# MicrobialDarkMatter/nanomotif

Hardware: AMD Instinct MI355X
Metric: motif-sites scored/sec (1 Gbp synthetic metagenome) (higher is better)
Workload: dtype u32 bit-planes / int64 counts

## Files before the change

### nanomotif_amd/csrc/nmscan.hip

```cpp
#define NM_SCORE_KERNEL_SOURCE
#include "nmscan_device.h"

using namespace nmdetail;

namespace {

thread_local std::string g_err;

__global__ __launch_bounds__(256) void pack_kernel(const uint8_t *__restrict__ ascii,
                                                   const uint64_t *__restrict__ contig_src,
                                                   const uint64_t *__restrict__ contig_len,
                                                   const uint32_t *__restrict__ chunk_contig,
                                                   const uint32_t *__restrict__ chunk_first,
                                                   uint32_t *__restrict__ H, uint32_t *__restrict__ L,
                                                   uint32_t *__restrict__ V, unsigned long long *__restrict__ other) {
    const uint32_t chunk = blockIdx.x;
    const uint32_t contig = chunk_contig[chunk];
    if (contig == 0xFFFFFFFFu) return;
    const uint64_t beg = contig_src[contig], len = contig_len[contig];
    const uint64_t local0 = (uint64_t)(chunk - chunk_first[contig]) * CHUNK_BP;
    const int lane = threadIdx.x & 63, wave = threadIdx.x >> 6;
    for (int it = wave; it < CHUNK_BP / 64; it += 4) {
        const uint64_t p = local0 + (uint64_t)it * 64 + lane;
        uint8_t c = 0;
// ... 514 lines not shown
    if (rc) return rc;
    c->cur_stage->last_out = r.rq.d_out;
    c->cur_stage->last_stream = r.sst;
    c->last_score_stream = r.sst;
    c->timed = !c->ev_collect && r.timed_launch;
    c->launches += 1;
    c->last_wgs = p.last_wgs;
    c->last_compact = p.all_compact ? p.n_prog : 0;
    c->last_general = p.all_compact ? 0 : p.n_prog;
    if (r.rq.defer) {
        nmdetail::wait_set(c, wait_slot, nm_ctx::Waiting{r.hs + p.off_counts, p.out_bytes, c->cur_stage, true});
    } else if (p.via_stage) {
        HIP_TRY(hipEventSynchronize(c->cur_stage->busy));
        memcpy(r.rq.h_out, r.hs + p.off_counts, p.out_bytes);
    } else if (r.rq.h_out) {
        HIP_TRY(hipMemcpyAsync(r.rq.h_out, r.out, p.out_bytes, hipMemcpyDeviceToHost, c->stream));
        HIP_TRY(hipStreamSynchronize(c->stream));
    }
    return NM_OK;
}

PlanFacts plan_facts(const nm_ctx *c) {
    PlanFacts f;
    f.n_bins = c->n_bins;
    f.bin_nchunks = c->bin_nchunks.data();
    f.bin_chunk0 = c->bin_chunk0.data();
    f.bin_ncontigs = c->bin_ncontigs.data();
    static_assert(NM_MAX_MOD_SLOTS <= 32, "one bit per mod slot");
    for (int sl = 0; sl < NM_MAX_MOD_SLOTS; ++sl) {
        f.slot_present |= (c->slots[sl].present ? 1u : 0u) << sl;
        f.slot_is_c |= (c->slots[sl].canonical == 'C' ? 1u : 0u) << sl;
    }
    f.n_segments = c->n_segments;
    f.seg_chunks = c->seg_chunks;
    f.n_cus = c->n_cus;
    f.opt_no_lit = c->opt_no_lit;
    f.opt_no_cf = c->opt_no_cf;
    f.opt_no_inline = c->opt_no_inline;
    f.opt_fine = c->opt_fine;
    f.opt_split = c->opt_split;
    return f;
}

int score_impl(nm_ctx *c, const ScoreRequest &rq) {
    if (!c) return fail(NM_EINVAL, "ctx is NULL");
    if (!c->dH) return fail(NM_ESTATE, "nm_upload_contigs has not been called");
    nm_ctx::Waiting &wait_slot = rq.spec ? c->spec_wait[rq.flight] : c->score_wait[rq.flight];
    if (rq.defer) {
        if (wait_slot.open) return fail(NM_ESTATE, "nm_score_batch_begin: the previous batch has not been collected (nm_score_batch_end)");
        nmdetail::wait_set(c, wait_slot, nm_ctx::Waiting{nullptr, 0, nullptr, true});
    }
    if (rq.n_cand == 0) return NM_OK;
    HIP_TRY(hipSetDevice(c->device));
    const PlanFacts f = plan_facts(c);
    c->bucket.assign((size_t)NM_MAX_MOD_SLOTS * f.n_bins + 1, 0);
    c->bin_active.assign(f.n_bins, 0);
    ScorePlan p;
    if (plan_classify(p, rq, f, c->bucket.data(), c->bin_active.data())) return fail(p.status, "%s", p.err);
    plan_shape(p, rq, f);
    plan_layout(p, rq);
    int rc = ensure_stage(c, p.via_stage ? p.stage_end : p.total, 1);
    if (rc) return rc;
    ScoreRun r{rq, p};
    r.sst = rq.spec ? static_cast<hipStream_t>(rq.stream) : c->stream;
    r.laned = c->score_lanes == 2 && rq.d_out && !rq.h_out && !rq.defer;
    if (!r.laned && !rq.spec) {
// ... 18 lines not shown
        HIP_TRY(hipStreamSynchronize(c->stream));
        HIP_TRY(hipStreamSynchronize(c->copy_stream));
        HIP_TRY(nmdetail::sync_flight_streams(c));
        rc = join_lanes(c);
        if (rc) return rc;
        if (c->d_programs) (void)nmdetail::dev_free(c->d_programs);
        c->d_programs = nullptr;
        c->prog_cap_dw = 0;
        HIP_TRY(nmdetail::dev_malloc(&c->d_programs, p.prog_dw * 2 * 4 * NM_STAGE_RING));
        c->prog_cap_dw = p.prog_dw * 2;
    }
    r.d_prog = c->d_programs + (size_t)(c->cur_stage - c->stage) * c->prog_cap_dw;
    r.out = rq.spec ? reinterpret_cast<unsigned long long *>(r.ds + p.off_counts) : rq.d_out;
    if (!r.out) {
        if (c->counts_cap < p.out_rows) {
            if (c->d_counts) (void)nmdetail::dev_free(c->d_counts);
            c->d_counts = nullptr;
            c->counts_cap = 0;
            HIP_TRY(nmdetail::dev_malloc(&c->d_counts, (size_t)p.out_rows * 2 * sizeof(unsigned long long) * 2));
            c->counts_cap = (size_t)p.out_rows * 2;
        }
        r.out = c->d_counts;
    }
    rc = score_prepare(c, r, f.slot_is_c);
    if (rc) return rc;
    plan_geometry(p, f);
    ScoreArgs a{};
    a.seq = Planes{c->dH, c->dL, c->dV, c->d_needs_v};
    for (int s = 0; s < NM_MAX_MOD_SLOTS; ++s) {
        const ModSlot &ms = c->slots[s];
        a.st[s] = StatePlanes{ms.planes[0], ms.planes[1], ms.planes[2], ms.planes[3], ms.planes[4], ms.planes[5]};
        a.slot_is_c[s] = ms.canonical == 'C';
    }
    a.segments = p.own_segments ? reinterpret_cast<const uint4 *>(r.ds + p.off_segs) : c->d_segments;
    a.n_segments = p.n_segments;
    a.n_bins = c->n_bins;
    a.programs = r.d_prog;
    a.orig_index = reinterpret_cast<uint32_t *>(r.ds + p.off_orig);
    a.cand_range = reinterpret_cast<uint4 *>(r.ds + p.off_range);
    a.out = r.out;
    a.chunk_rank = c->d_chunk_rank;
    a.row_base = reinterpret_cast<const uint64_t *>(r.ds + p.off_rows);
    for (uint32_t i = 0; i < p.n_active; ++i) a.active_slot[i] = p.active[i];
    a.split_log2 = p.split_log2;
    a.pieces_per_run = p.pieces_per_run;
    a.fine_log2 = p.fine_log2;
    a.j_big = p.j_big;
    const LaunchShape shape{p.any_wide, p.all_compact, p.lit, p.cf, p.fuse, p.per_contig, p.classes};
    if (r.timed_launch && p.compile != PLAN_COMPILE_SPEC) HIP_TRY(hipEventRecord(r.e0, r.sst));
    if (p.n_prog) launch_score(a, p.gx, p.gy, shape, r.sst);
    HIP_TRY(hipGetLastError());
    if (r.timed_launch) HIP_TRY(hipEventRecord(r.e1, r.sst));
    return score_collect(c, r, wait_slot);
}

}

int nm_set_error(int code, const char *fmt, ...) {
    char buf[512];
    va_list ap;
    va_start(ap, fmt);
    vsnprintf(buf, sizeof buf, fmt, ap);
    va_end(ap);
    g_err = buf;
    return code;
}

// ... 33 lines not shown
    HIP_TRY(hipEventCreate(&c->ev0));
    HIP_TRY(hipEventCreate(&c->ev1));
    HIP_TRY(nmdetail::dev_malloc(&c->d_err, sizeof(unsigned int)));
    HIP_TRY(nmdetail::dev_malloc(&c->d_other, sizeof(unsigned long long)));
    return NM_OK;
}

int nm_ctx_create(int device, nm_ctx **out) {
    if (!out) return fail(NM_EINVAL, "out is NULL");
    *out = nullptr;
    int n = 0;
    HIP_TRY(hipGetDeviceCount(&n));
    if (device < 0 || device >= n) return fail(NM_EINVAL, "device %d not in 0..%d", device, n - 1);
    HIP_TRY(hipSetDevice(device));
    nm_ctx *c = new (std::nothrow) nm_ctx();
    if (!c) return fail(NM_ENOMEM, "out of host memory");
    c->device = device;
    c->stream = nullptr;
    nmdetail::g_live_ctx += 1;
    const int rc = ctx_init(c);
    if (rc != NM_OK) {
        const std::string keep = g_err;
        (void)nm_ctx_destroy(c);
        g_err = keep;
        return rc;
    }
    *out = c;
    return NM_OK;
}

static void free_assembly(nm_ctx *c) {
    drop_ingest_rows(c);
    nmdetail::free_readstats(c);
    void *ptrs[] = {c->dH , c->d_needs_v, c->d_contig_chunk, c->d_contig_len, c->d_segments, c->d_chunk_rank};
    c->d_chunk_rank = nullptr;
    for (void *p : ptrs)
        if (p) (void)nmdetail::dev_free(p);
    c->dH = c->dL = c->dV = nullptr;
    c->d_needs_v = nullptr;
    c->d_contig_chunk = nullptr;
    c->d_contig_len = nullptr;
    c->d_segments = nullptr;
    for (int b = 0; b < 4; ++b) {
        if (c->d_rank[b]) (void)nmdetail::dev_free(c->d_rank[b]);
        if (c->d_base_total[b]) (void)nmdetail::dev_free(c->d_base_total[b]);
        c->d_rank[b] = nullptr;
        c->d_base_total[b] = nullptr;
    }
    for (auto &s : c->slots) {
        free_slot_planes(s);
        s.present = false;
        s.n_rows = 0;
        drop_slot_ranks(s);
    }
}

int nm_ctx_destroy(nm_ctx *c) {
    if (!c) return NM_OK;
    (void)hipSetDevice(c->device);
    if (c->stream) (void)hipStreamSynchronize(c->stream);
    if (c->own_stream) (void)hipStreamSynchronize(c->own_stream);
    if (c->copy_stream) (void)hipStreamSynchronize(c->copy_stream);
    if (c->lane_stream) (void)hipStreamSynchronize(c->lane_stream);
    c->lane_pending = false;
    (void)nm_comm_destroy(c);
    free_assembly(c);
    for (auto &st : c->stage) {
        if (st.d) (void)nmdetail::dev_free(st.d);
// ... 138 lines not shown
        guard.tmp[0] = d_ascii;
    }
    HIP_TRY(nmdetail::dev_malloc(&d_off, (size_t)(n_contigs + 1) * 8));
    guard.tmp[1] = d_off;
    HIP_TRY(nmdetail::dev_malloc(&d_chunk_contig, (size_t)c->n_chunks * 4));
    guard.tmp[2] = d_chunk_contig;
    if (!on_device && c->total_bp) HIP_TRY(hipMemcpyAsync(d_ascii, seq_ascii, c->total_bp, hipMemcpyHostToDevice, c->stream));
    HIP_TRY(hipMemcpyAsync(d_off, src_off ? src_off : offsets, (size_t)(n_contigs + (src_off ? 0 : 1)) * 8, hipMemcpyHostToDevice, c->stream));
    HIP_TRY(hipMemcpyAsync(d_chunk_contig, chunk_contig.data(), (size_t)c->n_chunks * 4, hipMemcpyHostToDevice, c->stream));
    {
        std::vector<uint32_t> chunk_rank(c->n_chunks, 0);
        for (uint32_t ch = 0; ch < c->n_chunks; ++ch)
            if (chunk_contig[ch] != 0xFFFFFFFFu) chunk_rank[ch] = c->contig_rank[chunk_contig[ch]];
        HIP_TRY(nmdetail::dev_malloc(&c->d_chunk_rank, (size_t)c->n_chunks * 4));
        HIP_TRY(hipMemcpy(c->d_chunk_rank, chunk_rank.data(), (size_t)c->n_chunks * 4, hipMemcpyHostToDevice));
    }
    HIP_TRY(hipMemsetAsync(c->d_other, 0, sizeof(unsigned long long), c->stream));
    hipLaunchKernelGGL(pack_kernel, dim3(c->n_chunks), dim3(256), 0, c->stream, d_ascii, d_off, c->d_contig_len, d_chunk_contig,
                       c->d_contig_chunk, c->dH, c->dL, c->dV, c->d_other);
    HIP_TRY(hipGetLastError());
    hipLaunchKernelGGL(needs_v_kernel, dim3(c->n_chunks), dim3(CHUNK_WORDS), 0, c->stream, c->dV, c->d_needs_v, c->n_chunks);
    HIP_TRY(hipGetLastError());
    std::vector<uint4> segs;
    for (uint32_t b = 0; b < n_bins; ++b)
        for (uint32_t k = 0; k < c->bin_nchunks[b]; k += c->seg_chunks)
            segs.push_back(make_uint4(c->bin_chunk0[b] + k, std::min<uint32_t>(c->seg_chunks, c->bin_nchunks[b] - k), b, 0));
    c->n_segments = (uint32_t)segs.size();
    HIP_TRY(nmdetail::dev_malloc(&c->d_segments, std::max<size_t>(segs.size(), 1) * sizeof(uint4)));
    if (!segs.empty()) HIP_TRY(hipMemcpyAsync(c->d_segments, segs.data(), segs.size() * sizeof(uint4), hipMemcpyHostToDevice, c->stream));
    unsigned long long other = 0;
    HIP_TRY(hipMemcpyAsync(&other, c->d_other, sizeof other, hipMemcpyDeviceToHost, c->stream));
    HIP_TRY(hipStreamSynchronize(c->stream));
    c->other_letters = other;
    guard.keep = true;
    return NM_OK;
}

static int upload_pileup_impl(nm_ctx *c, uint32_t mod_slot, uint8_t canonical_base, double low, double high,
                              uint64_t n_rows, const uint32_t *contig_id, const uint32_t *position,
                              const uint8_t *strand, const double *fraction_mod, int append, bool on_device) {
    if (!c) return fail(NM_EINVAL, "ctx is NULL");
    if (!c->dH) return fail(NM_ESTATE, "nm_upload_contigs must come first");
    if (mod_slot >= NM_MAX_MOD_SLOTS) return fail(NM_EINVAL, "mod_slot %u >= %d", mod_slot, NM_MAX_MOD_SLOTS);
    if (canonical_base != 'A' && canonical_base != 'C') return fail(NM_EINVAL, "canonical base must be 'A' or 'C'");
    if (!(high > low)) return fail(NM_EINVAL, "high threshold must exceed low (find_motifs_bin.py:117-118)");
    if (n_rows && (!contig_id || !position || !strand || !fraction_mod)) return fail(NM_EINVAL, "NULL column");
    HIP_TRY(hipSetDevice(c->device));
    HIP_TRY(hipStreamSynchronize(c->stream));
    {
        const int rcj = join_lanes(c);
        if (rcj) return rcj;
    }
    ModSlot &ms = c->slots[mod_slot];
    drop_slot_ranks(ms);
    const size_t words = plane_words(c);
    if (!ms.present || !append) {
        HIP_TRY(alloc_slot_planes(ms, words));
        HIP_TRY(hipMemsetAsync(ms.planes[0], 0, words * 4 * 6, c->stream));
        ms.n_rows = 0;
    } else if (ms.canonical != canonical_base || ms.low != low || ms.high != high) {
        return fail(NM_EINVAL, "append with different canonical base / thresholds than the slot holds");
    }
    ms.present = true;
    ms.canonical = canonical_base;
    ms.low = low;
    ms.high = high;
// ... 447 lines not shown
```

### nanomotif_amd/csrc/nmscan_device.h

```cpp
#pragma once
#include "nmscan_internal.h"

namespace nmdetail {

__device__ __forceinline__ uint32_t alignbit(uint32_t hi, uint32_t lo, uint32_t sh) {
    return __builtin_amdgcn_alignbit(hi, lo, sh);
}

typedef const uint32_t __attribute__((address_space(4))) *cu32p;
typedef const uint8_t __attribute__((address_space(4))) *cu8p;

#ifndef NM_LIT_WAVES
#define NM_LIT_WAVES 4
#endif

template <int GN_, int GP_, bool COMPACT_, int NS_, bool LIT_, bool CF_, bool PC_ = false, bool CLS_ = false>
struct Variant {
    static constexpr int GN = GN_, GP = GP_, NS = NS_;
    static constexpr bool COMPACT = COMPACT_, LIT = LIT_, CF = CF_, PC = PC_;
    static constexpr bool CLS = CLS_;
    static_assert(!CLS || (GN == 1 && GP == 1 && COMPACT && NS == 1 && !LIT && !CF), "class planes: narrow compact heavy variants only");
    static constexpr int NW = T_WORDS + GN + GP;
    static constexpr int NP = LIT ? 4 : 8;
    static constexpr int NST = COMPACT ? 2 : 4;
    static constexpr int PDW = (GN + GP) * NP;
};

template <class K>
struct RawChunk {
    uint32_t h[K::NW], l[K::NW], v[K::NW];
    uint32_t s[K::NS][K::NST][T_WORDS];
    bool need_v;

    __device__ __forceinline__ void load(const Planes &seq, const StatePlanes (&stp)[K::NS], uint32_t chunk, int lane) {
        constexpr int GN = K::GN, GP = K::GP;
        need_v = ((cu8p)seq.needs_v)[chunk] != 0;
        const size_t base = (size_t)chunk * CHUNK_WORDS + (size_t)lane * T_WORDS;
#pragma unroll
        for (int j = 0; j < K::NS; ++j) {
            const uint32_t *src[4] = {K::COMPACT ? stp[j].M : stp[j].MP, K::COMPACT ? stp[j].U : stp[j].UP, stp[j].MM, stp[j].UM};
#pragma unroll
            for (int i = 0; i < K::NST; ++i) {
                const uint4 q = *reinterpret_cast<const uint4 *>(src[i] + base);
                s[j][i][0] = q.x; s[j][i][1] = q.y; s[j][i][2] = q.z; s[j][i][3] = q.w;
            }
        }
        const uint4 h4 = *reinterpret_cast<const uint4 *>(seq.H + base);
        const uint4 l4 = *reinterpret_cast<const uint4 *>(seq.L + base);
        h[GN + 0] = h4.x; h[GN + 1] = h4.y; h[GN + 2] = h4.z; h[GN + 3] = h4.w;
        l[GN + 0] = l4.x; l[GN + 1] = l4.y; l[GN + 2] = l4.z; l[GN + 3] = l4.w;
#pragma unroll
        for (int j = 0; j < GN; ++j) { h[j] = seq.H[base - GN + j]; l[j] = seq.L[base - GN + j]; }
#pragma unroll
        for (int j = 0; j < GP; ++j) { h[GN + T_WORDS + j] = seq.H[base + T_WORDS + j]; l[GN + T_WORDS + j] = seq.L[base + T_WORDS + j]; }
        if (need_v) {
            const uint4 v4 = *reinterpret_cast<const uint4 *>(seq.V + base);
            v[GN + 0] = v4.x; v[GN + 1] = v4.y; v[GN + 2] = v4.z; v[GN + 3] = v4.w;
#pragma unroll
            for (int j = 0; j < GN; ++j) v[j] = seq.V[base - GN + j];
#pragma unroll
            for (int j = 0; j < GP; ++j) v[GN + T_WORDS + j] = seq.V[base + T_WORDS + j];
        } else if constexpr (!K::CLS) {
#pragma unroll
            for (int j = 0; j < K::NW; ++j) v[j] = 0xFFFFFFFFu;
        }
    }
};

template <class K>
struct Tile {
// ... 405 lines not shown
                    prog[1] = desc[1];
                }
                r.w = 1;
            }
            r.z = n_prog + g;
        }
    }
    range[g] = r;
}


}

#ifdef NM_SCORE_KERNEL_SOURCE

namespace nmdetail {

struct ScoreArgs {
    Planes seq;
    StatePlanes st[NM_MAX_MOD_SLOTS];
    const uint4 *segments;
    uint32_t n_segments;
    uint32_t split_log2;
    uint32_t pieces_per_run, j_big, fine_log2;
    uint32_t n_bins;
    const uint4 *cand_range;
    const uint32_t *programs;
    const uint32_t *orig_index;
    unsigned long long *out;
    const uint32_t *chunk_rank;
    const uint64_t *row_base;
    uint32_t active_slot[NM_MAX_MOD_SLOTS];
    uint32_t slot_is_c[NM_MAX_MOD_SLOTS];
};

void launch_score_classes(const ScoreArgs &a, uint32_t gx, uint32_t gy, bool per_contig, hipStream_t s);

}

namespace {

using namespace nmdetail;

template <class K, int I = 0>
__device__ __forceinline__ void apply_single(uint32_t idx, uint32_t r, const Tile<K> &tile, const uint32_t (&base)[T_WORDS],
                                             uint32_t (&acc)[T_WORDS]) {
    if constexpr (I < K::PDW) {
        if (idx == I) {
            constexpr int g = I / K::NP, p = I % K::NP;
#pragma unroll
            for (int t = 0; t < T_WORDS; ++t) acc[t] = base[t] & alignbit(tile.w[p][t + g + 1], tile.w[p][t + g], r);
        } else {
            apply_single<K, I + 1>(idx, r, tile, base, acc);
        }
    } else {
#pragma unroll
        for (int t = 0; t < T_WORDS; ++t) acc[t] = base[t];
    }
}

template <class K>
__device__ __forceinline__ void emit_counts(const ScoreArgs &a, uint32_t n_mod, uint32_t n_non, uint32_t k0, uint32_t k,
                                            uint32_t *lds_acc, uint32_t lds_row0, int lane, uint32_t contig_rank) {
    if (K::PC) {
        if constexpr (K::CLS) {
#define NM_SWZ_ADD(o)                                                                         \
// ... 197 lines not shown
            const uint32_t i = idx >> 2, q = idx & 3;
            const uint32_t j = (i >> 1) % NS, k = (i >> 1) / NS;
            uint32_t s = 0;
#pragma unroll 4
            for (int jj = 0; jj < 16; ++jj) s += lds_acc[i * 64 + q * 16 + jj];
            s += __shfl_xor(s, 1);
            s += __shfl_xor(s, 2);
            if (q == 0 && s) {
                uint4 rj = range[0];
#pragma unroll
                for (int t = 1; t < NS; ++t)
                    if (j == (uint32_t)t) rj = range[t];
                if (pass0 + k < rj.y) {
                    const uint32_t orig = a.orig_index[rj.x + pass0 + k];
                    atomicAdd(a.out + (size_t)orig * 2 + (i & 1), (unsigned long long)s);
                }
            }
        }
        __syncthreads();
    };
    uint32_t pass0 = 0;
    if (EARLY) {
        const uint32_t rows_hi = NS * min(H, most);
        clear_rows(rows_hi);
        if (wave < sg.y) score_chunk(first, 0, sg.x + wave);
        for (uint32_t ck = wave + 4; ck < sg.y; ck += 4) {
            RawChunk<K> cur;
            cur.load(a.seq, stp, sg.x + ck, lane);
            score_chunk(cur, 0, sg.x + ck);
        }
        flush_rows(rows_hi, 0);
        pass0 = H;
    }
    for (; pass0 < most; pass0 += H) {
        const uint32_t rows_hi = NS * min(H, most - pass0);
        clear_rows(rows_hi);
        for (uint32_t ck = wave; ck < sg.y; ck += 4) {
            RawChunk<K> cur;
            cur.load(a.seq, stp, sg.x + ck, lane);
            score_chunk(cur, pass0, sg.x + ck);
        }
        flush_rows(rows_hi, pass0);
    }
}

#define NM_SCORE_BOUNDS __launch_bounds__(256, (K::GN + K::GP > 2 ? 2 : (K::LIT ? NM_LIT_WAVES : (K::CLS ? 6 : 4))))

#define NM_SLOT_SETUP                                                                                               \
    const int lane = threadIdx.x & 63;                                                                              \
    const uint32_t wave = __builtin_amdgcn_readfirstlane(threadIdx.x >> 6);  \
    StatePlanes stp[K::NS];                                                                                         \
    bool is_c[K::NS];                                                                                               \
    _Pragma("unroll") for (int j = 0; j < K::NS; ++j) {                                                             \
        const uint32_t slot = a.active_slot[K::NS == 1 ? blockIdx.y : (uint32_t)j];                                 \
        stp[j] = a.st[slot];                                                                                        \
        is_c[j] = a.slot_is_c[slot] != 0;                                                                           \
    }

template <class K>
__global__ NM_SCORE_BOUNDS void score_kernel(ScoreArgs a) {
    __shared__ uint32_t lds_acc[BMAX * 2 * 64];
    const uint32_t lanes_x = K::CF ? 1u : 8u;
    const uint32_t x = K::CF ? 0u : blockIdx.x % 8, j = K::CF ? blockIdx.x : blockIdx.x / 8;
    uint32_t piece, sub = 0, n_sub = 1;
    if (j < a.j_big) piece = x * a.pieces_per_run + j;
    else {
        const uint32_t k = j - a.j_big;
        piece = x * a.pieces_per_run + a.j_big + (k >> a.fine_log2);
        sub = k & ((1u << a.fine_log2) - 1);
        n_sub = 1u << a.fine_log2;
        if (a.j_big + (k >> a.fine_log2) >= a.pieces_per_run) return;
    }
    (void)lanes_x;
    const uint32_t seg = piece >> a.split_log2;
    if (seg >= a.n_segments) return;
    uint4 sg = a.segments[seg];
    sg.x = __builtin_amdgcn_readfirstlane(sg.x);
    sg.y = __builtin_amdgcn_readfirstlane(sg.y);
    sg.z = __builtin_amdgcn_readfirstlane(sg.z);
    if (a.split_log2) {
        const uint32_t len = (sg.y + (1u << a.split_log2) - 1) >> a.split_log2;
        const uint32_t at = (piece & ((1u << a.split_log2) - 1)) * len;
        if (at >= sg.y) return;
        sg.x += at;
        sg.y = min(len, sg.y - at);
    }
    if (n_sub > 1) {
        const uint32_t len = (sg.y + n_sub - 1) / n_sub;
        const uint32_t at = sub * len;
        if (at >= sg.y) return;
        sg.x += at;
        sg.y = min(len, sg.y - at);
    }
    NM_SLOT_SETUP
    score_piece<K>(a, sg, stp, is_c, lds_acc, lane, wave);
}

}

#ifdef NM_SCORE_CLASSES_UNIT
namespace nmdetail {

void launch_score_classes(const ScoreArgs &a, uint32_t gx, uint32_t gy, bool per_contig, hipStream_t s) {
    if (per_contig) hipLaunchKernelGGL((score_kernel<Variant<1, 1, true, 1, false, false, true, true>>), dim3(gx, gy), dim3(256), 0, s, a);
    else hipLaunchKernelGGL((score_kernel<Variant<1, 1, true, 1, false, false, false, true>>), dim3(gx, gy), dim3(256), 0, s, a);
}

}
#endif

#endif
```

### nanomotif_amd/csrc/nmscan_internal.h

```cpp
#pragma once
#include <hip/hip_runtime.h>

#include <algorithm>
#include <cstdarg>
#include <cstdint>
#include <cstdio>
#include <cstring>
#include <functional>
#include <mutex>
#include <numeric>
#include <string>
#include <vector>

#include "../../include/nmscan.h"
#include "nmscore_plan.h"
#include "nmspec.h"

int nm_set_error(int code, const char *fmt, ...);
#define fail nm_set_error

#define HIP_TRY(expr)                                                                                   \
    do {                                                                                                \
        hipError_t e_ = (expr);                                                                         \
        if (e_ != hipSuccess) return fail(NM_EHIP, "%s failed: %s", #expr, hipGetErrorString(e_));      \
    } while (0)

namespace nmdetail {

hipError_t device_alloc(void **p, size_t bytes);
hipError_t device_free(void *p);
template <class T>
inline hipError_t dev_malloc(T **p, size_t bytes) { return device_alloc(reinterpret_cast<void **>(p), bytes); }
inline hipError_t dev_free(void *p) { return device_free(p); }

constexpr int T_WORDS = 4;
constexpr int CHUNK_WORDS = 64 * T_WORDS;
constexpr int CHUNK_BP = CHUNK_WORDS * 32;
constexpr int GAP_BP = 96;
constexpr int SEG_CHUNKS = 16;
constexpr int BMAX = 32;
constexpr int NM_MAX_MOD_CODES = 8;
constexpr int NM_CODE_STRIDE = 128;
constexpr int WIN_MAX_W = NM_WIN_MAX_WIDTH;
constexpr int RANK_BLOCK_WORDS = 16;
constexpr int RANK_PER_CHUNK = CHUNK_WORDS / RANK_BLOCK_WORDS;

struct Planes {
    const uint32_t *H, *L, *V;
// ... 48 lines not shown
    hipStream_t last_score_stream = nullptr;
    std::vector<uint32_t> bucket;
    std::vector<uint8_t> bin_active;
    std::vector<nmdetail::WinTask> win_tasks;
    uint32_t *d_win_planes = nullptr, *d_win_alive = nullptr;
    uint64_t win_planes_cap = 0, win_alive_cap = 0, win_planes_used = 0, win_alive_used = 0;
    nmdetail::WinTask *d_win_tasks = nullptr;
    size_t d_win_tasks_cap = 0;
    bool win_tasks_dirty = false;
    std::vector<uint32_t> ing_kept;
    int ing_slot_of_mod[8] = {-1, -1, -1, -1, -1, -1, -1, -1};
    uint64_t ing_nconf = 0, ing_total_kept = 0, ing_classified = 0;
    uint32_t *d_programs = nullptr;
    size_t prog_cap_dw = 0;
    hipEvent_t ev0 = nullptr, ev1 = nullptr;
    bool timed = false;
    std::vector<std::pair<hipEvent_t, hipEvent_t>> ev_pool;
    size_t ev_used = 0;
    bool ev_collect = false;
    bool busy_open = false;
    bool ev_collect_all = false;
    uint32_t n_contigs = 0, n_bins = 0, n_chunks = 0;
    uint64_t total_bp = 0;
    std::vector<uint64_t> contig_len;
    std::vector<uint32_t> contig_chunk, contig_bin, contig_nchunks;
    std::vector<uint32_t> bin_chunk0, bin_nchunks, bin_ncontigs, contig_rank;
    uint32_t *d_chunk_rank = nullptr;
    uint32_t *dH = nullptr, *dL = nullptr, *dV = nullptr;
    uint8_t *d_needs_v = nullptr;
    uint32_t *d_contig_chunk = nullptr;
    uint64_t *d_contig_len = nullptr;
    uint4 *d_segments = nullptr;
    uint32_t n_segments = 0;
    nmdetail::ModSlot slots[NM_MAX_MOD_SLOTS];
    nmdetail::ReadStats readstats[NM_MAX_MOD_SLOTS];
    uint32_t *d_chunk_contig = nullptr;
    struct Stage {
        void *d = nullptr, *h = nullptr;
        size_t bytes = 0;
        hipEvent_t busy = nullptr;
        bool pending = false;
        const void *last_out = nullptr;
        hipStream_t last_stream = nullptr;
    } stage[NM_STAGE_SLOTS];
    int stage_next = 0;
    int stage_next_deep = 0;
    void *d_stage = nullptr, *h_stage = nullptr;
    Stage *cur_stage = nullptr;
    struct Waiting {
        const void *h = nullptr;
        size_t bytes = 0;
        Stage *stage = nullptr;
        bool open = false;
    } score_wait[NM_FLIGHTS], win_wait[NM_FLIGHTS], spec_wait[NM_FLIGHTS];
    std::mutex wait_mu;
    hipStream_t flight_stream[NM_FLIGHTS - 1] = {};
    double *d_spec_bg = nullptr;
    uint32_t spec_tasks = 0, spec_width = 0;
    unsigned long long *d_spec_counts[NM_FLIGHTS] = {}, *d_flight_counts[NM_FLIGHTS] = {};
    size_t spec_counts_cap[NM_FLIGHTS] = {}, flight_counts_cap[NM_FLIGHTS] = {};
    unsigned long long *d_counts = nullptr;
    size_t counts_cap = 0;
    unsigned int *d_err = nullptr;
    uint32_t *d_rank[4] = {nullptr, nullptr, nullptr, nullptr};
    uint64_t *d_base_total[4] = {nullptr, nullptr, nullptr, nullptr};
    unsigned long long *d_other = nullptr;
// ... 121 lines not shown
```

### nanomotif_amd/csrc/nmscore_plan.h

```cpp
#pragma once
#include <algorithm>
#include <cstdarg>
#include <cstddef>
#include <cstdint>
#include <cstdio>
#include <cstdlib>
#include <cstring>

#include "../../include/nmscan.h"

namespace nmdetail {

struct SpecSource;

struct CandRec {
    uint32_t mask_off;
    uint32_t orig;
    uint8_t len, modpos, slot, pad;
};

struct PlanU4 { uint32_t x, y, z, w; };

constexpr size_t PLAN_STAGE_DIRECT_MAX = (size_t)4 << 20;

struct ScoreRequest {
    uint32_t n_cand = 0;
    const uint32_t *bin = nullptr;
    const uint8_t *slot = nullptr, *len = nullptr, *modpos = nullptr;
    const uint32_t *mask_off = nullptr;
    const uint8_t *masks = nullptr;
    unsigned long long *d_out = nullptr;
    int64_t *h_out = nullptr;
    const uint64_t *row_offset = nullptr;
    bool defer = false;
    const SpecSource *spec = nullptr;
    uint32_t spec_mask_stride = 0;
    size_t spec_extra_in = 0, spec_extra_out = 0;
    void *stream = nullptr;
    int flight = 0;
};

struct PlanFacts {
    uint32_t n_bins = 0;
    const uint32_t *bin_nchunks = nullptr, *bin_chunk0 = nullptr, *bin_ncontigs = nullptr;
    uint32_t slot_present = 0, slot_is_c = 0;
    uint32_t n_segments = 0, seg_chunks = 16, n_cus = 256;
    bool opt_no_lit = false, opt_no_cf = false, opt_no_inline = false;
    int opt_fine = -1, opt_split = -1;
};

enum PlanCompile { PLAN_COMPILE_NONE, PLAN_COMPILE_FUSED, PLAN_COMPILE_ONLY, PLAN_COMPILE_THEN_COMMON, PLAN_COMPILE_SPEC };

struct ScorePlan {
    int status = NM_OK;
    char err[192] = {0};
    int any_wide = 0;
    bool all_compact = true, all_literal = true, per_contig = false;
    uint32_t n_prog = 0;
    uint64_t mask_lo = 0, mask_hi = 0;
    uint32_t n_active = 0, active[NM_MAX_MOD_SLOTS] = {};
    int slot_to_active[NM_MAX_MOD_SLOTS] = {};
    uint32_t n_active_bins = 0, n_groups = 0;
    size_t n_active_segs = 0;
    uint64_t out_rows = 0;
    bool lit = false, light = false, cf = false, classes = false, cls_head = true, fuse = false;
    bool own_segments = false, via_stage = false, inline_prep = false, by_kernels = false;
    PlanCompile compile = PLAN_COMPILE_NONE;
    uint32_t np = 8, pdw = 0, n_entries = 0;
    size_t prog_dw = 0;
    size_t off_orig = 0, off_masks = 0, off_range = 0, off_rows = 0, off_segs = 0, off_posof = 0, off_xin = 0, total = 0;
    size_t off_counts = 0, off_xout = 0, stage_end = 0;
    size_t range_bytes = 0, out_bytes = 0, clear_bytes = 0;
    uint32_t n_segments = 0;
    uint32_t split_log2 = 0, pieces_per_run = 0, fine_log2 = 0, j_big = 0, gx = 0, gy = 1;
    uint64_t last_wgs = 0;
};

inline size_t plan_align16(size_t x) { return (x + 15) & ~(size_t)15; }

inline int plan_fail(ScorePlan &p, int code, const char *fmt, ...) __attribute__((format(printf, 3, 4)));
inline int plan_fail(ScorePlan &p, int code, const char *fmt, ...) {
    va_list ap;
    va_start(ap, fmt);
    vsnprintf(p.err, sizeof p.err, fmt, ap);
    va_end(ap);
    return p.status = code;
}

inline int check_motif(ScorePlan &p, uint32_t k, uint32_t len, uint32_t mp, const uint8_t *m, uint32_t max_len, bool *literal) {
    if (len == 0 || len > max_len) return plan_fail(p, NM_ERANGE, "candidate %u: motif length %u outside 1..%d", k, len, (int)max_len);
    if (mp >= len) return plan_fail(p, NM_EINVAL, "candidate %u: mod_position %u outside motif of length %u", k, mp, len);
    uint32_t all_and = 15u, any_zero = 0, any_set = 0;
    for (uint32_t j = 0; j < len; ++j) {
        const uint32_t v = m[j] & 15u;
        all_and &= v;
        any_zero |= (v == 0);
        any_set |= (v != 15u) & ((v & (v - 1)) != 0);
    }
    if (any_zero) return plan_fail(p, NM_EINVAL, "candidate %u: empty base set in the motif", k);
    if (all_and == 15u) return plan_fail(p, NM_EINVAL, "candidate %u: motif has no specified position", k);
    *literal = !any_set;
    return NM_OK;
}

inline uint32_t number_active_slots(const bool used[NM_MAX_MOD_SLOTS], int slot_to_active[NM_MAX_MOD_SLOTS], uint32_t *active = nullptr) {
    uint32_t n = 0;
    for (int s = 0; s < NM_MAX_MOD_SLOTS; ++s) {
        slot_to_active[s] = -1;
        if (!used[s]) continue;
        if (active) active[n] = (uint32_t)s;
        slot_to_active[s] = (int)n++;
    }
    return n;
}

inline int plan_classify(ScorePlan &p, const ScoreRequest &rq, const PlanFacts &f, uint32_t *bucket, uint8_t *bin_active) {
    const uint32_t n_bins = f.n_bins;
    uint64_t mask_bytes = 0, mask_lo = ~0ull;
    bool slot_used[NM_MAX_MOD_SLOTS] = {};
    for (uint32_t k = 0; k < rq.n_cand; ++k) {
        const uint32_t slot = rq.slot[k], bin = rq.bin[k];
        if (slot >= NM_MAX_MOD_SLOTS || !(f.slot_present >> slot & 1u))
            return plan_fail(p, NM_ESTATE, "candidate %u uses mod slot %u with no pileup uploaded", k, slot);
        if (bin >= n_bins) return plan_fail(p, NM_EINVAL, "candidate %u: bin %u >= n_bins %u", k, bin, n_bins);
        if (f.bin_nchunks[bin] == 0) continue;
        if (rq.spec) {
            mask_lo = 0;
            mask_bytes = std::max<uint64_t>(mask_bytes, (uint64_t)(k + 1) * rq.spec_mask_stride);
        } else {
            const uint32_t len = rq.len[k], mp = rq.modpos[k];
            const uint8_t *m = rq.masks + rq.mask_off[k];
            bool literal = true;
            if (check_motif(p, k, len, mp, m, NM_MAX_MOTIF_LEN, &literal)) return p.status;
            if (!literal) p.all_literal = false;
            mask_lo = std::min<uint64_t>(mask_lo, rq.mask_off[k]);
            mask_bytes = std::max<uint64_t>(mask_bytes, (uint64_t)rq.mask_off[k] + len);
            const uint32_t reach = std::max(mp, len - 1 - mp);
            if (reach > 95) return plan_fail(p, NM_ERANGE, "candidate %u: a position %u away from the modified base (the engine reaches 95)", k, reach);
            p.any_wide = std::max(p.any_wide, reach > 63 ? 2 : reach > 31 ? 1 : 0);
            if ((m[mp] & 15u) != ((f.slot_is_c >> slot & 1u) ? NM_BASE_C : NM_BASE_A)) p.all_compact = false;
        }
        bucket[(size_t)slot * n_bins + bin + 1] += 1;
        slot_used[slot] = true;
        p.n_prog += 1;
    }
    if (p.n_prog == 0) { mask_lo = 0; mask_bytes = 0; }
    p.mask_lo = mask_lo;
    p.mask_hi = mask_bytes;
    p.n_active = number_active_slots(slot_used, p.slot_to_active, p.active);
    p.per_contig = rq.row_offset != nullptr;
    p.out_rows = p.per_contig ? rq.row_offset[rq.n_cand] : rq.n_cand;
    if (p.per_contig)
        for (uint32_t k = 0; k < rq.n_cand; ++k)
            if (rq.row_offset[k + 1] - rq.row_offset[k] != f.bin_ncontigs[rq.bin[k]])
                return plan_fail(p, NM_EINVAL, "candidate %u: %llu output rows for a bin of %u resident contigs", k,
                                 (unsigned long long)(rq.row_offset[k + 1] - rq.row_offset[k]), f.bin_ncontigs[rq.bin[k]]);
    for (uint32_t b = 0; b < n_bins; ++b) {
        uint32_t groups = 0;
        for (uint32_t i = 0; i < p.n_active; ++i) groups += bucket[(size_t)p.active[i] * n_bins + b + 1] > 0;
        if (!groups) continue;
        p.n_groups += groups;
        bin_active[b] = 1;
        p.n_active_bins += 1;
        p.n_active_segs += (f.bin_nchunks[b] + f.seg_chunks - 1) / f.seg_chunks;
    }
    return NM_OK;
}

inline void plan_shape(ScorePlan &p, const ScoreRequest &rq, const PlanFacts &f) {
    p.lit = p.all_literal && p.all_compact && !p.any_wide && !f.opt_no_lit && !p.per_contig;
    p.np = p.lit ? 4u : 8u;
    p.pdw = 2u * (2u + 2u * (uint32_t)p.any_wide) * p.np;
    p.light = (uint64_t)p.n_prog <= 6ull * p.n_groups && !p.per_contig;
    p.cf = p.light && !f.opt_no_cf;
    p.fuse = p.n_active == 2 && p.cf && p.lit;
    const char *cls_env = getenv("NM_SCORE_CLASSES"), *head_env = getenv("NM_SCORE_HEAD");
    p.cls_head = !(head_env && atoi(head_env) == 0);
    p.classes = !rq.spec && !p.lit && !p.any_wide && p.all_compact && !p.cf && !(cls_env && atoi(cls_env) == 0);
    p.own_segments = p.n_prog && p.n_active_segs * 4 <= (size_t)f.n_segments * 3 && getenv("NM_ALL_SEGMENTS") == nullptr;
    p.n_segments = p.own_segments ? (uint32_t)p.n_active_segs : f.n_segments;
    p.n_entries = std::max(p.n_active, 1u) * f.n_bins;
    p.prog_dw = ((size_t)std::max(p.n_prog, 1u) + (p.cf ? p.n_entries : 0)) * p.pdw;
    p.out_bytes = (size_t)p.out_rows * 2 * sizeof(int64_t);
    p.via_stage = rq.defer || (rq.h_out && p.out_bytes <= PLAN_STAGE_DIRECT_MAX);
    p.inline_prep = (rq.h_out || rq.defer) && !f.opt_no_inline;
    if (rq.spec) p.compile = PLAN_COMPILE_SPEC;
    else if (!p.n_prog) p.compile = PLAN_COMPILE_NONE;
    else if (p.cf && p.n_prog <= 2048 && p.n_entries <= 8192 && !f.opt_no_inline) p.compile = PLAN_COMPILE_FUSED;
    else p.compile = p.cf ? PLAN_COMPILE_THEN_COMMON : PLAN_COMPILE_ONLY;
}

inline void plan_layout(ScorePlan &p, const ScoreRequest &rq) {
    const size_t rec_bytes = (size_t)p.n_prog * sizeof(CandRec);
    p.off_orig = plan_align16(rec_bytes);
    p.off_masks = plan_align16(p.off_orig + (size_t)p.n_prog * 4);
    p.off_range = plan_align16(p.off_masks + (p.mask_hi - p.mask_lo));
    p.range_bytes = (size_t)p.n_entries * sizeof(PlanU4);
    p.off_rows = plan_align16(p.off_range + p.range_bytes);
    const size_t rows_end = p.off_rows + (p.per_contig ? (size_t)p.n_prog * 8 : 0);
    p.off_segs = plan_align16(rows_end);
    const size_t segs_end = p.own_segments ? p.off_segs + p.n_active_segs * sizeof(PlanU4) : p.off_segs;
    p.off_posof = plan_align16(segs_end);
    p.off_xin = plan_align16(p.off_posof + (size_t)rq.n_cand * 4);
    p.total = rq.spec ? p.off_xin + rq.spec_extra_in : p.own_segments ? segs_end : rows_end;
    p.off_counts = plan_align16(p.total);
    p.off_xout = plan_align16(p.off_counts + p.out_bytes);
    p.stage_end = rq.spec ? p.off_xout + rq.spec_extra_out : p.off_counts + p.out_bytes;
    p.clear_bytes = rq.spec ? p.stage_end - p.off_counts : (size_t)p.out_rows * 2 * sizeof(unsigned long long);
    p.by_kernels = p.inline_prep && p.total <= PLAN_STAGE_DIRECT_MAX && (p.via_stage || !rq.h_out) && getenv("NM_STAGE_COPIES") == nullptr;
}

inline void plan_fill(const ScorePlan &p, const ScoreRequest &rq, const PlanFacts &f, uint32_t *bucket, const uint8_t *bin_active, uint8_t *hs) {
    const uint32_t n_bins = f.n_bins;
    CandRec *h_rec = reinterpret_cast<CandRec *>(hs);
    uint32_t *h_orig = reinterpret_cast<uint32_t *>(hs + p.off_orig);
    PlanU4 *h_range = reinterpret_cast<PlanU4 *>(hs + p.off_range);
    if (!rq.spec && p.mask_hi > p.mask_lo) memcpy(hs + p.off_masks, rq.masks + p.mask_lo, p.mask_hi - p.mask_lo);
    memset(h_range, 0, p.range_bytes);
    if (p.own_segments) {
        PlanU4 *h_segs = reinterpret_cast<PlanU4 *>(hs + p.off_segs);
        size_t at = 0;
        for (uint32_t b = 0; b < n_bins; ++b)
            if (bin_active[b])
                for (uint32_t k = 0; k < f.bin_nchunks[b]; k += f.seg_chunks)
                    h_segs[at++] = PlanU4{f.bin_chunk0[b] + k, std::min<uint32_t>(f.seg_chunks, f.bin_nchunks[b] - k), b, 0};
    }
    const size_t n_bucket = (size_t)NM_MAX_MOD_SLOTS * n_bins + 1;
    for (size_t i = 1; i < n_bucket; ++i) bucket[i] += bucket[i - 1];
    for (uint32_t i = 0; i < p.n_active; ++i)
        for (uint32_t b = 0; b < n_bins; ++b) {
            const uint32_t lo = bucket[(size_t)p.active[i] * n_bins + b], hi = bucket[(size_t)p.active[i] * n_bins + b + 1];
            if (hi > lo) h_range[(size_t)i * n_bins + b] = PlanU4{lo, hi - lo, 0xFFFFFFFFu, 0};
        }
    for (uint32_t k = 0; k < rq.n_cand; ++k) {
        const uint32_t slot = rq.slot[k], bin = rq.bin[k];
        if (f.bin_nchunks[bin] == 0) continue;
        const uint32_t at = bucket[(size_t)slot * n_bins + bin]++;
        h_orig[at] = k;
        if (rq.spec) {
            h_rec[at] = CandRec{k * rq.spec_mask_stride, k, 0, 0, (uint8_t)slot, 0};
            reinterpret_cast<uint32_t *>(hs + p.off_posof)[k] = at;
            continue;
        }
        h_rec[at] = CandRec{(uint32_t)(rq.mask_off[k] - p.mask_lo), k, rq.len[k], rq.modpos[k], (uint8_t)slot, 0};
        if (p.per_contig) reinterpret_cast<uint64_t *>(hs + p.off_rows)[at] = rq.row_offset[k];
    }
}

inline void plan_geometry(ScorePlan &p, const PlanFacts &f) {
    uint64_t est_wgs = (uint64_t)p.n_segments * p.n_groups / std::max<uint32_t>(p.own_segments ? p.n_active_bins : f.n_bins, 1);
    if (p.light && p.n_active == 2 && p.lit) est_wgs = (est_wgs + 1) / 2;
    const uint64_t resident = (uint64_t)f.n_cus * 6;
    uint32_t split_log2 = 0;
    while (split_log2 < 2 && (est_wgs << split_log2) < 2 * resident) ++split_log2;
    if (f.opt_split >= 0) split_log2 = (uint32_t)f.opt_split;
    p.split_log2 = split_log2;
    const uint32_t runs = p.cf ? 1u : 8u;
    const uint32_t n_pieces = p.n_segments << split_log2;
// ... 12 lines not shown
```

Before: 102900 billion.

## Score chunks through a prebuilt work list that packs partial contig tails

At upload time a work list is built for each bin. It drops chunks lying wholly in contig padding and, by default, packs the partially filled tail chunks of short contigs into dense 64-strip rows, with one strip per lane. The non-CF, non-per-contig scoring path reads each chunk through this list, indirecting per lane for packed rows, so waves stop scanning empty bit-plane padding. The cost is an extra host-side build and a device allocation at upload, plus one more indirection in the kernel. Packed rows force need_v on, and segment geometry now depends on the list.

```diff
diff --git a/nanomotif_amd/csrc/nmscan.hip b/nanomotif_amd/csrc/nmscan.hip
--- a/nanomotif_amd/csrc/nmscan.hip
+++ b/nanomotif_amd/csrc/nmscan.hip
@@ -570,6 +570,11 @@
         f.slot_is_c |= (c->slots[sl].canonical == 'C' ? 1u : 0u) << sl;
     }
     f.n_segments = c->n_segments;
+    for (int w = 0; w < 2; ++w) {
+        f.list_start[w] = c->list_start[w].data();
+        f.list_len[w] = c->list_len[w].data();
+        f.list_segments[w] = c->n_list_segments[w];
+    }
     f.seg_chunks = c->seg_chunks;
     f.n_cus = c->n_cus;
     f.opt_no_lit = c->opt_no_lit;
@@ -654,7 +659,9 @@
         a.st[s] = StatePlanes{ms.planes[0], ms.planes[1], ms.planes[2], ms.planes[3], ms.planes[4], ms.planes[5]};
         a.slot_is_c[s] = ms.canonical == 'C';
     }
-    a.segments = p.own_segments ? reinterpret_cast<const uint4 *>(r.ds + p.off_segs) : c->d_segments;
+    a.segments = p.own_segments ? reinterpret_cast<const uint4 *>(r.ds + p.off_segs) : p.use_list ? c->d_list_segments[p.pack] : c->d_segments;
+    a.work_list = c->d_work_list[p.pack];
+    a.strip_rows = c->d_strip_rows;
     a.n_segments = p.n_segments;
     a.n_bins = c->n_bins;
     a.programs = r.d_prog;
@@ -754,8 +761,17 @@
 static void free_assembly(nm_ctx *c) {
     drop_ingest_rows(c);
     nmdetail::free_readstats(c);
-    void *ptrs[] = {c->dH , c->d_needs_v, c->d_contig_chunk, c->d_contig_len, c->d_segments, c->d_chunk_rank};
+    void *ptrs[] = {c->dH , c->d_needs_v, c->d_contig_chunk, c->d_contig_len, c->d_segments, c->d_chunk_rank,
+                    c->d_work_list[0] };
     c->d_chunk_rank = nullptr;
+    for (int w = 0; w < 2; ++w) {
+        c->d_work_list[w] = nullptr;
+        c->d_list_segments[w] = nullptr;
+        c->n_list_segments[w] = 0;
+        c->list_start[w].clear();
+        c->list_len[w].clear();
+    }
+    c->d_strip_rows = nullptr;
     for (void *p : ptrs)
         if (p) (void)nmdetail::dev_free(p);
     c->dH = c->dL = c->dV = nullptr;
@@ -960,6 +976,33 @@
     HIP_TRY(hipMemcpyAsync(&other, c->d_other, sizeof other, hipMemcpyDeviceToHost, c->stream));
     HIP_TRY(hipStreamSynchronize(c->stream));
     c->other_letters = other;
+    {
+        std::vector<uint8_t> needs_v(c->n_chunks);
+        HIP_TRY(hipMemcpy(needs_v.data(), c->d_needs_v, c->n_chunks, hipMemcpyDeviceToHost));
+        WorkList wl[2];
+        for (int w = 0; w < 2; ++w)
+            build_work_list(wl[w], w == 1, n_bins, n_contigs, order.data(), c->contig_bin.data(), c->contig_len.data(), c->contig_chunk.data(), needs_v.data(),
+                            c->n_chunks, c->seg_chunks);
+        const size_t o_list[2] = {0, wl[0].entries.size()}, o_strips = o_list[1] + wl[1].entries.size();
+        const size_t o_segs0 = (o_strips + wl[1].strip_rows.size() + 3) & ~(size_t)3, o_segs1 = o_segs0 + wl[0].segs.size() * 4;
+        const size_t o_segs[2] = {o_segs0, o_segs1}, total = o_segs1 + wl[1].segs.size() * 4;
+        std::vector<uint32_t> blob(std::max<size_t>(total, 4), 0);
+        for (int w = 0; w < 2; ++w) {
+            std::copy(wl[w].entries.begin(), wl[w].entries.end(), blob.begin() + o_list[w]);
+            if (!wl[w].segs.empty()) memcpy(blob.data() + o_segs[w], wl[w].segs.data(), wl[w].segs.size() * sizeof(PlanU4));
+        }
+        std::copy(wl[1].strip_rows.begin(), wl[1].strip_rows.end(), blob.begin() + o_strips);
+        HIP_TRY(nmdetail::dev_malloc(&c->d_work_list[0], blob.size() * 4));
+        HIP_TRY(hipMemcpy(c->d_work_list[0], blob.data(), blob.size() * 4, hipMemcpyHostToDevice));
+        c->d_work_list[1] = c->d_work_list[0] + o_list[1];
+        c->d_strip_rows = c->d_work_list[0] + o_strips;
+        for (int w = 0; w < 2; ++w) {
+            c->d_list_segments[w] = reinterpret_cast<uint4 *>(c->d_work_list[0] + o_segs[w]);
+            c->n_list_segments[w] = (uint32_t)wl[w].segs.size();
+            c->list_start[w] = std::move(wl[w].bin_start);
+            c->list_len[w] = std::move(wl[w].bin_len);
+        }
+    }
     guard.keep = true;
     return NM_OK;
 }
diff --git a/nanomotif_amd/csrc/nmscan_device.h b/nanomotif_amd/csrc/nmscan_device.h
--- a/nanomotif_amd/csrc/nmscan_device.h
+++ b/nanomotif_amd/csrc/nmscan_device.h
@@ -33,9 +33,21 @@
     bool need_v;
 
     __device__ __forceinline__ void load(const Planes &seq, const StatePlanes (&stp)[K::NS], uint32_t chunk, int lane) {
+        need_v = ((cu8p)seq.needs_v)[chunk] != 0;
+        load_at(seq, stp, (size_t)chunk * CHUNK_WORDS + (size_t)lane * T_WORDS);
+    }
+    __device__ __forceinline__ void load_entry(const Planes &seq, const StatePlanes (&stp)[K::NS], uint32_t entry, const uint32_t *strip_rows, int lane) {
+        if (entry & WORK_PACKED) {
+            const uint32_t w = strip_rows[(size_t)(entry & ~WORK_PACKED) * WORK_STRIPS + lane];
+            need_v = true;
+            load_at(seq, stp, (size_t)(w == WORK_NO_STRIP ? (uint32_t)T_WORDS : w));
+        } else {
+            need_v = (entry & WORK_NEED_V) != 0;
+            load_at(seq, stp, (size_t)(entry & (WORK_NEED_V - 1)) * CHUNK_WORDS + (size_t)lane * T_WORDS);
+        }
+    }
+    __device__ __forceinline__ void load_at(const Planes &seq, const StatePlanes (&stp)[K::NS], const size_t base) {
         constexpr int GN = K::GN, GP = K::GP;
-        need_v = ((cu8p)seq.needs_v)[chunk] != 0;
-        const size_t base = (size_t)chunk * CHUNK_WORDS + (size_t)lane * T_WORDS;
 #pragma unroll
         for (int j = 0; j < K::NS; ++j) {
             const uint32_t *src[4] = {K::COMPACT ? stp[j].M : stp[j].MP, K::COMPACT ? stp[j].U : stp[j].UP, stp[j].MM, stp[j].UM};
@@ -507,6 +519,8 @@
     const uint64_t *row_base;
     uint32_t active_slot[NM_MAX_MOD_SLOTS];
     uint32_t slot_is_c[NM_MAX_MOD_SLOTS];
+    const uint32_t *work_list;
+    const uint32_t *strip_rows;
 };
 
 void launch_score_classes(const ScoreArgs &a, uint32_t gx, uint32_t gy, bool per_contig, hipStream_t s);
@@ -770,13 +784,15 @@
         flush_rows(rows_hi, 0);
         pass0 = H;
     }
+    constexpr bool LIST = !K::CF && !K::PC;
     for (; pass0 < most; pass0 += H) {
         const uint32_t rows_hi = NS * min(H, most - pass0);
         clear_rows(rows_hi);
         for (uint32_t ck = wave; ck < sg.y; ck += 4) {
             RawChunk<K> cur;
-            cur.load(a.seq, stp, sg.x + ck, lane);
-            score_chunk(cur, pass0, sg.x + ck);
+            if constexpr (LIST) cur.load_entry(a.seq, stp, ((cu32p)a.work_list)[sg.x + ck], a.strip_rows, lane);
+            else cur.load(a.seq, stp, sg.x + ck, lane);
+            score_chunk(cur, pass0, LIST ? 0u : sg.x + ck);
         }
         flush_rows(rows_hi, pass0);
     }
@@ -798,38 +814,20 @@
 template <class K>
 __global__ NM_SCORE_BOUNDS void score_kernel(ScoreArgs a) {
     __shared__ uint32_t lds_acc[BMAX * 2 * 64];
-    const uint32_t lanes_x = K::CF ? 1u : 8u;
-    const uint32_t x = K::CF ? 0u : blockIdx.x % 8, j = K::CF ? blockIdx.x : blockIdx.x / 8;
-    uint32_t piece, sub = 0, n_sub = 1;
-    if (j < a.j_big) piece = x * a.pieces_per_run + j;
+    const PlanGrid grid{a.n_segments, a.split_log2, a.pieces_per_run, a.j_big, a.fine_log2};
+    uint32_t piece, sub, n_sub;
+    if (!plan_block_piece(grid, K::CF, blockIdx.x, &piece, &sub, &n_sub)) return;
+    typedef const uint4 __attribute__((address_space(4))) *cu4p;
+    uint4 sg;
+    if constexpr (K::CF) sg = a.segments[piece >> a.split_log2];
     else {
-        const uint32_t k = j - a.j_big;
-        piece = x * a.pieces_per_run + a.j_big + (k >> a.fine_log2);
-        sub = k & ((1u << a.fine_log2) - 1);
-        n_sub = 1u << a.fine_log2;
-        if (a.j_big + (k >> a.fine_log2) >= a.pieces_per_run) return;
-    }
-    (void)lanes_x;
-    const uint32_t seg = piece >> a.split_log2;
-    if (seg >= a.n_segments) return;
-    uint4 sg = a.segments[seg];
+        const cu4p seg = (cu4p)a.segments + (piece >> a.split_log2);
+        sg.x = seg->x; sg.y = seg->y; sg.z = seg->z; sg.w = 0;
+    }
     sg.x = __builtin_amdgcn_readfirstlane(sg.x);
     sg.y = __builtin_amdgcn_readfirstlane(sg.y);
     sg.z = __builtin_amdgcn_readfirstlane(sg.z);
-    if (a.split_log2) {
-        const uint32_t len = (sg.y + (1u << a.split_log2) - 1) >> a.split_log2;
-        const uint32_t at = (piece & ((1u << a.split_log2) - 1)) * len;
-        if (at >= sg.y) return;
-        sg.x += at;
-        sg.y = min(len, sg.y - at);
-    }
-    if (n_sub > 1) {
-        const uint32_t len = (sg.y + n_sub - 1) / n_sub;
-        const uint32_t at = sub * len;
-        if (at >= sg.y) return;
-        sg.x += at;
-        sg.y = min(len, sg.y - at);
-    }
+    if (!plan_cut_piece(grid, piece, sub, n_sub, &sg.x, &sg.y)) return;
     NM_SLOT_SETUP
     score_piece<K>(a, sg, stp, is_c, lds_acc, lane, wave);
 }
diff --git a/nanomotif_amd/csrc/nmscan_internal.h b/nanomotif_amd/csrc/nmscan_internal.h
--- a/nanomotif_amd/csrc/nmscan_internal.h
+++ b/nanomotif_amd/csrc/nmscan_internal.h
@@ -14,6 +14,7 @@
 
 #include "../../include/nmscan.h"
 #include "nmscore_plan.h"
+#include "nmscore_worklist.h"
 #include "nmspec.h"
 
 int nm_set_error(int code, const char *fmt, ...);
@@ -128,6 +129,10 @@
     uint64_t *d_contig_len = nullptr;
     uint4 *d_segments = nullptr;
     uint32_t n_segments = 0;
+    uint32_t *d_work_list[2] = {nullptr, nullptr}, *d_strip_rows = nullptr;
+    uint4 *d_list_segments[2] = {nullptr, nullptr};
+    uint32_t n_list_segments[2] = {0, 0};
+    std::vector<uint32_t> list_start[2], list_len[2];
     nmdetail::ModSlot slots[NM_MAX_MOD_SLOTS];
     nmdetail::ReadStats readstats[NM_MAX_MOD_SLOTS];
     uint32_t *d_chunk_contig = nullptr;
diff --git a/nanomotif_amd/csrc/nmscore_plan.h b/nanomotif_amd/csrc/nmscore_plan.h
--- a/nanomotif_amd/csrc/nmscore_plan.h
+++ b/nanomotif_amd/csrc/nmscore_plan.h
@@ -47,6 +47,8 @@
     uint32_t n_segments = 0, seg_chunks = 16, n_cus = 256;
     bool opt_no_lit = false, opt_no_cf = false, opt_no_inline = false;
     int opt_fine = -1, opt_split = -1;
+    const uint32_t *list_start[2] = {nullptr, nullptr}, *list_len[2] = {nullptr, nullptr};
+    uint32_t list_segments[2] = {0, 0};
 };
 
 enum PlanCompile { PLAN_COMPILE_NONE, PLAN_COMPILE_FUSED, PLAN_COMPILE_ONLY, PLAN_COMPILE_THEN_COMMON, PLAN_COMPILE_SPEC };
@@ -62,6 +64,7 @@
     int slot_to_active[NM_MAX_MOD_SLOTS] = {};
     uint32_t n_active_bins = 0, n_groups = 0;
     size_t n_active_segs = 0;
+    bool use_list = false, pack = false;
     uint64_t out_rows = 0;
     bool lit = false, light = false, cf = false, classes = false, cls_head = true, fuse = false;
     bool own_segments = false, via_stage = false, inline_prep = false, by_kernels = false;
@@ -78,6 +81,54 @@
 
 inline size_t plan_align16(size_t x) { return (x + 15) & ~(size_t)15; }
 
+#if defined(__HIPCC__)
+#define NM_PLAN_HD __host__ __device__ __forceinline__
+#else
+#define NM_PLAN_HD inline
+#endif
+
+struct PlanGrid { uint32_t n_segments, split_log2, pieces_per_run, j_big, fine_log2; };
+
+NM_PLAN_HD bool plan_block_piece(const PlanGrid &g, bool cf, uint32_t block, uint32_t *piece, uint32_t *sub, uint32_t *n_sub) {
+    const uint32_t x = cf ? 0u : block % 8, j = cf ? block : block / 8;
+    *sub = 0;
+    *n_sub = 1;
+    if (j < g.j_big) *piece = x * g.pieces_per_run + j;
+    else {
+        const uint32_t k = j - g.j_big;
+        *piece = x * g.pieces_per_run + g.j_big + (k >> g.fine_log2);
+        *sub = k & ((1u << g.fine_log2) - 1);
+        *n_sub = 1u << g.fine_log2;
+        if (g.j_big + (k >> g.fine_log2) >= g.pieces_per_run) return false;
+    }
+    return (*piece >> g.split_log2) < g.n_segments;
+}
+NM_PLAN_HD bool plan_cut_piece(const PlanGrid &g, uint32_t piece, uint32_t sub, uint32_t n_sub, uint32_t *first, uint32_t *count) {
+    if (g.split_log2) {
+        const uint32_t len = (*count + (1u << g.split_log2) - 1) >> g.split_log2;
+        const uint32_t at = (piece & ((1u << g.split_log2) - 1)) * len;
+        if (at >= *count) return false;
+        *first += at;
+        *count = len < *count - at ? len : *count - at;
+    }
+    if (n_sub > 1) {
+        const uint32_t len = (*count + n_sub - 1) / n_sub;
+        const uint32_t at = sub * len;
+        if (at >= *count) return false;
+        *first += at;
+        *count = len < *count - at ? len : *count - at;
+    }
+    return true;
+}
+inline bool plan_decode_block(const PlanGrid &g, bool cf, uint32_t block, const PlanU4 *segments, uint32_t *seg, uint32_t *first, uint32_t *count) {
+    uint32_t piece, sub, n_sub;
+    if (!plan_block_piece(g, cf, block, &piece, &sub, &n_sub)) return false;
+    *seg = piece >> g.split_log2;
+    *first = segments[*seg].x;
+    *count = segments[*seg].y;
+    return plan_cut_piece(g, piece, sub, n_sub, first, count);
+}
+
 inline int plan_fail(ScorePlan &p, int code, const char *fmt, ...) __attribute__((format(printf, 3, 4)));
 inline int plan_fail(ScorePlan &p, int code, const char *fmt, ...) {
     va_list ap;
@@ -113,6 +164,8 @@
     }
     return n;
 }
+
+inline bool plan_is_light(const ScorePlan &p) { return (uint64_t)p.n_prog <= 6ull * p.n_groups && !p.per_contig; }
 
 inline int plan_classify(ScorePlan &p, const ScoreRequest &rq, const PlanFacts &f, uint32_t *bucket, uint8_t *bin_active) {
     const uint32_t n_bins = f.n_bins;
@@ -155,6 +208,9 @@
             if (rq.row_offset[k + 1] - rq.row_offset[k] != f.bin_ncontigs[rq.bin[k]])
                 return plan_fail(p, NM_EINVAL, "candidate %u: %llu output rows for a bin of %u resident contigs", k,
                                  (unsigned long long)(rq.row_offset[k + 1] - rq.row_offset[k]), f.bin_ncontigs[rq.bin[k]]);
+    const char *pack_env = getenv("NM_SCORE_PACK_TAILS");
+    const int which = pack_env && atoi(pack_env) == 0 ? 0 : 1;
+    size_t list_segs = 0;
     for (uint32_t b = 0; b < n_bins; ++b) {
         uint32_t groups = 0;
         for (uint32_t i = 0; i < p.n_active; ++i) groups += bucket[(size_t)p.active[i] * n_bins + b + 1] > 0;
@@ -163,7 +219,11 @@
         bin_active[b] = 1;
         p.n_active_bins += 1;
         p.n_active_segs += (f.bin_nchunks[b] + f.seg_chunks - 1) / f.seg_chunks;
-    }
+        if (f.list_len[which]) list_segs += (f.list_len[which][b] + f.seg_chunks - 1) / f.seg_chunks;
+    }
+    p.use_list = f.list_len[which] && !p.per_contig && !(plan_is_light(p) && !f.opt_no_cf);
+    p.pack = p.use_list && which == 1;
+    if (p.use_list) p.n_active_segs = list_segs;
     return NM_OK;
 }
 
@@ -171,14 +231,15 @@
     p.lit = p.all_literal && p.all_compact && !p.any_wide && !f.opt_no_lit && !p.per_contig;
     p.np = p.lit ? 4u : 8u;
     p.pdw = 2u * (2u + 2u * (uint32_t)p.any_wide) * p.np;
-    p.light = (uint64_t)p.n_prog <= 6ull * p.n_groups && !p.per_contig;
+    p.light = plan_is_light(p);
     p.cf = p.light && !f.opt_no_cf;
     p.fuse = p.n_active == 2 && p.cf && p.lit;
     const char *cls_env = getenv("NM_SCORE_CLASSES"), *head_env = getenv("NM_SCORE_HEAD");
     p.cls_head = !(head_env && atoi(head_env) == 0);
     p.classes = !rq.spec && !p.lit && !p.any_wide && p.all_compact && !p.cf && !(cls_env && atoi(cls_env) == 0);
-    p.own_segments = p.n_prog && p.n_active_segs * 4 <= (size_t)f.n_segments * 3 && getenv("NM_ALL_SEGMENTS") == nullptr;
-    p.n_segments = p.own_segments ? (uint32_t)p.n_active_segs : f.n_segments;
+    const uint32_t static_segments = p.use_list ? f.list_segments[p.pack] : f.n_segments;
+    p.own_segments = p.n_prog && p.n_active_segs * 4 <= (size_t)static_segments * 3 && getenv("NM_ALL_SEGMENTS") == nullptr;
+    p.n_segments = p.own_segments ? (uint32_t)p.n_active_segs : static_segments;
     p.n_entries = std::max(p.n_active, 1u) * f.n_bins;
     p.prog_dw = ((size_t)std::max(p.n_prog, 1u) + (p.cf ? p.n_entries : 0)) * p.pdw;
     p.out_bytes = (size_t)p.out_rows * 2 * sizeof(int64_t);
@@ -219,11 +280,12 @@
     memset(h_range, 0, p.range_bytes);
     if (p.own_segments) {
         PlanU4 *h_segs = reinterpret_cast<PlanU4 *>(hs + p.off_segs);
+        const uint32_t *first = p.use_list ? f.list_start[p.pack] : f.bin_chunk0, *count = p.use_list ? f.list_len[p.pack] : f.bin_nchunks;
         size_t at = 0;
         for (uint32_t b = 0; b < n_bins; ++b)
             if (bin_active[b])
-                for (uint32_t k = 0; k < f.bin_nchunks[b]; k += f.seg_chunks)
-                    h_segs[at++] = PlanU4{f.bin_chunk0[b] + k, std::min<uint32_t>(f.seg_chunks, f.bin_nchunks[b] - k), b, 0};
+                for (uint32_t k = 0; k < count[b]; k += f.seg_chunks)
+                    h_segs[at++] = PlanU4{first[b] + k, std::min<uint32_t>(f.seg_chunks, count[b] - k), b, 0};
     }
     const size_t n_bucket = (size_t)NM_MAX_MOD_SLOTS * n_bins + 1;
     for (size_t i = 1; i < n_bucket; ++i) bucket[i] += bucket[i - 1];
diff --git a/nanomotif_amd/csrc/nmscore_worklist.h b/nanomotif_amd/csrc/nmscore_worklist.h
--- /dev/null
+++ b/nanomotif_amd/csrc/nmscore_worklist.h
@@ -0,0 +1,56 @@
+#pragma once
+#include <cstdint>
+#include <vector>
+
+#include "nmscore_plan.h"
+
+namespace nmdetail {
+
+constexpr uint32_t WORK_CHUNK_BP = 8192, WORK_STRIP_BP = 128, WORK_STRIPS = 64, WORK_CHUNK_WORDS = 256, WORK_GAP_BP = 96;
+constexpr uint32_t WORK_NEED_V = 1u << 30, WORK_PACKED = 1u << 31, WORK_NO_STRIP = 0xFFFFFFFFu;
+
+struct WorkList {
+    std::vector<uint32_t> entries;
+    std::vector<uint32_t> strip_rows;
+    std::vector<PlanU4> segs;
+    std::vector<uint32_t> bin_start, bin_len;
+};
+
+inline uint32_t work_strips_of(uint64_t len, uint64_t q) {
+    const uint64_t at = q * WORK_CHUNK_BP;
+    if (len <= at) return 0;
+    return (uint32_t)std::min<uint64_t>(WORK_STRIPS, (len - at + WORK_STRIP_BP - 1) / WORK_STRIP_BP);
+}
+
+inline void build_work_list(WorkList &wl, bool pack, uint32_t n_bins, uint32_t n_contigs, const uint32_t *order, const uint32_t *contig_bin,
+                            const uint64_t *contig_len, const uint32_t *contig_chunk, const uint8_t *needs_v, uint32_t n_chunks, uint32_t seg_chunks) {
+    if ((uint64_t)n_chunks * WORK_CHUNK_WORDS > 0xFFFFFFFFull) pack = false;
+    wl.entries.clear();
+    wl.strip_rows.clear();
+    wl.segs.clear();
+    wl.bin_start.assign(n_bins, 0);
+    wl.bin_len.assign(n_bins, 0);
+    uint32_t oi = 0;
+    for (uint32_t b = 0; b < n_bins; ++b) {
+        const uint32_t start = (uint32_t)wl.entries.size();
+        const size_t row0 = wl.strip_rows.size() / WORK_STRIPS;
+        for (; oi < n_contigs && contig_bin[order[oi]] == b; ++oi) {
+            const uint32_t i = order[oi];
+            const uint64_t nch = (contig_len[i] + WORK_GAP_BP + WORK_CHUNK_BP - 1) / WORK_CHUNK_BP;
+            for (uint64_t q = 0; q < nch; ++q) {
+                const uint32_t chunk = contig_chunk[i] + (uint32_t)q, strips = work_strips_of(contig_len[i], q);
+                if (strips == 0) continue;
+                if (!pack || strips == WORK_STRIPS) wl.entries.push_back(chunk | (needs_v[chunk] ? WORK_NEED_V : 0u));
+                else for (uint32_t s = 0; s < strips; ++s) wl.strip_rows.push_back(chunk * WORK_CHUNK_WORDS + s * 4);
+            }
+        }
+        while (wl.strip_rows.size() % WORK_STRIPS) wl.strip_rows.push_back(WORK_NO_STRIP);
+        for (size_t row = row0; row < wl.strip_rows.size() / WORK_STRIPS; ++row) wl.entries.push_back(WORK_PACKED | (uint32_t)row);
+        wl.bin_start[b] = start;
+        wl.bin_len[b] = (uint32_t)wl.entries.size() - start;
+        for (uint32_t k = 0; k < wl.bin_len[b]; k += seg_chunks)
+            wl.segs.push_back(PlanU4{start + k, std::min<uint32_t>(seg_chunks, wl.bin_len[b] - k), b, 0});
+    }
+}
+
+}
```

New measurement: 104900 billion (median of 6 runs). 1.02x the previous value.
